# BreakTheBeta/Zonos_Vibes

Measured on AMD Instinct MI355X. Metric: real-time factor (44kHz audio s/compute s) + DAC tokens/s/GPU, Zonos-transformer, higher is better.
Workload: dtype bf16; 1 GPU; C2: batch=1 per GPU, Lc=160, 861 frames (10.00 s audio), greedy + rep. penalty, EOS suppressed, + DAC decode; global_batch=1, seq_len=1030, parallelism=dp1 (utterance-sharded), decode_steps=869

## Files before the change

include/zonos_hip.h:

```cpp
#ifndef ZONOS_HIP_H
#define ZONOS_HIP_H
#include <stdint.h>

#ifdef __cplusplus
extern "C" {
#endif

enum {
  ZMI_EPI_STORE = 0,
  ZMI_EPI_RESIDUAL = 1,
  ZMI_EPI_QKV = 2,
  ZMI_EPI_SWIGLU = 3,
  ZMI_EPI_LOGITS = 4,
  ZMI_EPI_F32 = 5
};
enum { ZMI_PACK_IDENTITY = 0, ZMI_PACK_SWIGLU = 1 };
enum { ZMI_PRO_AUTO = 0, ZMI_PRO_ADDLN = 2, ZMI_PRO_GRMS = 3, ZMI_PRO_GRMS_G = 4 };
enum { ZMI_WFMT_BF16 = 0, ZMI_WFMT_FP8 = 1 };

typedef struct ZmiGemvArgs {
  const void* W;
  const void* X;
  int M, N, K, ldx;
  int groups;
// ... 30 lines not shown
  int n_cb, n_rt, rpw;
} ZmiGemvForm;
int zmi_gemv_form(const ZmiGemvArgs* args, int epi, ZmiGemvForm* out);
int zmi_gemv_splitk(const ZmiGemvArgs* args, int epi, float* part, int64_t part_floats, void* stream);
int zmi_gemv_splitk_ln(const ZmiGemvArgs* args, int epi, float* part, int64_t part_floats, const void* ln_w,
                       const void* ln_b, float eps, void* xn, int ldxn, void* stream);
int64_t zmi_gemv_splitk_floats(int M, int N);
int zmi_layernorm_rows(const void* x, int ldx, int m, int k, const void* w, const void* b, float eps, void* out,
                       int ldo, void* stream);

int zmi_attention(const void* q, int ldq, const void* k_cache, const void* v_cache, const int* q_kv_row,
                  const int* q_pos, int n_query, int hq, int hkv, int hd, int smax, int max_pos, void* out,
                  int ldo, float* part_o, float* part_lm, void* work, void* stream);
int zmi_attention_variant(const void* q, int ldq, const void* k_cache, const void* v_cache, const int* q_kv_row,
                          const int* q_pos, int n_query, int hq, int hkv, int hd, int smax, int max_pos, void* out,
                          int ldo, float* part_o, float* part_lm, void* work, int variant, void* stream);
int zmi_attention_max_keys_whole(void);
int zmi_attention_pick(int n_query, int hkv, int variant);
int zmi_attn_block(const ZmiGemvArgs* qkv, void* gran, unsigned* err, void* attn_out, int ldo, int slices,
                   void* stream);
enum { ZMI_ATTNBLK_SELF = 256, ZMI_ATTNBLK_SPLIT = 512 };
int zmi_attn_block_max_pos(int slices);
int64_t zmi_attn_block_gran_words(int rows, int hkv);
typedef struct ZmiPrefetch {
  const void* ptr[2];
  int64_t bytes[2];
  unsigned* sink;
  int blocks, reserved;
} ZmiPrefetch;
int zmi_attn_block_pf(const ZmiGemvArgs* qkv, void* gran, unsigned* err, void* attn_out, int ldo, int slices,
                      const ZmiPrefetch* prefetch, void* stream);
int zmi_attn_block_oproj(const ZmiGemvArgs* qkv, const ZmiGemvArgs* oproj, void* gran, unsigned* err, void* attn_out,
                         int ldo, int slices, const ZmiPrefetch* prefetch, void* stream);
int zmi_attention_pf(const void* q, int ldq, const void* k_cache, const void* v_cache, const int* q_kv_row,
                     const int* q_pos, int n_query, int hq, int hkv, int hd, int smax, int max_pos, void* out, int ldo,
                     float* part_o, float* part_lm, void* work, int variant, const ZmiPrefetch* prefetch,
                     void* stream);
int64_t zmi_attention_work_bytes(int n_query, int hq, int hkv, int hd, int max_pos);
int64_t zmi_attention_partial_floats(int n_query, int hq, int hkv, int hd, int max_pos);
int zmi_attention_chunk(void);
typedef struct ZmiAttnSeq { int q_row0, len, kv_row, pos0; } ZmiAttnSeq;
typedef struct ZmiAttnTile { int seq, off; } ZmiAttnTile;
int zmi_attention_prefill(const void* q, int ldq, const void* k_cache, const void* v_cache, const ZmiAttnSeq* seqs,
                          int n_seq, int64_t n_tiles, const ZmiAttnTile* tiles, const ZmiAttnSeq* seqs_host, int hq,
                          int hkv, int hd, int smax, void* out, int ldo, void* stream);
int zmi_attention_prefill_queries(int hq, int hkv);

typedef struct ZmiSampling {
  float temperature, top_p, min_p, linear, conf, quad, rep_penalty, cfg_scale;
  int top_k, rep_window;
  uint64_t seed;
} ZmiSampling;

typedef struct ZmiSlots {
  int* active;
  int* pos;
  int* offset;
  int* remaining;
  int* stopping;
  int* step;
  int* delayed;
  const ZmiSampling* params;
  const int* total_len;
  int tcap;
  int n_slots;
} ZmiSlots;
// ... 123 lines not shown
  void* conv_ring;
  void* ssm;
  void* y;
  int ldy, gz_g;
  const int* row_pos;
  const int* row_kv;
  float* gz;
} ZmiMamba2Args;
int zmi_mamba2_step(const ZmiMamba2Args* args, void* stream);
int zmi_mamba2_scan(const ZmiMamba2Args* args, int seq_len, void* stream);
int zmi_mamba2_scan_ws(const ZmiMamba2Args* args, int seq_len, void* ws, int64_t ws_bytes, void* stream);
int64_t zmi_mamba2_scan_ws_bytes(int m, int d_ssm, int nheads);
int zmi_mamba2_scan_seqs(const ZmiMamba2Args* args, const ZmiAttnSeq* seqs, int n_seq, const ZmiAttnSeq* seqs_host,
                         void* ws, int64_t ws_bytes, void* stream);
int zmi_add_layernorm(const void* hidden, int ldh, void* residual, int ldr, int m, int k, const void* w,
                      const void* b, float eps, void* out, int ldo, int store_residual, void* stream);
int zmi_gated_rmsnorm(const void* y, int ldy, const void* z, int ldz, int m, int k, const void* w, float eps,
                      void* out, int ldo, void* stream);
int zmi_mamba_block(const ZmiGemvArgs* in_proj, const ZmiMamba2Args* step, void* gran, unsigned* err, void* stream);
int64_t zmi_mamba_block_gran_words(int rows, int d_in_proj);
int zmi_mamba_block_pf(const ZmiGemvArgs* in_proj, const ZmiMamba2Args* step, void* gran, unsigned* err,
                       const ZmiPrefetch* prefetch, void* stream);

int zmi_fill_uniform(void* dst, int64_t n, uint64_t key, float scale, float offset, int dtype, void* stream);

int zmi_graph_begin(void* stream);
int zmi_graph_end(void* stream, void** graph_exec);
int zmi_graph_launch(void* graph_exec, int times, void* stream);
int zmi_graph_destroy(void* graph_exec);

const char* zmi_last_error(void);
int zmi_version(void);
int zmi_xcd_dealing(void* stream);
enum { ZMI_OPT_GEMV_SPREAD = 0, ZMI_OPT_GEMM_ROWS = 1, ZMI_OPT_XC_HANDOFF = 2,
       ZMI_OPT_DAC_WIDE = 10, ZMI_OPT_DAC_WIDE_MIN = 11, ZMI_OPT_ATTNBLK_SPREAD = 12, ZMI_OPT_DAC_STAGE = 13,
       ZMI_OPT_DAC_STAGE_MIN = 14, ZMI_OPT_SCAN_PQ = 15, ZMI_OPT_SPLITK_WGS = 16, ZMI_OPT_SPLITK_STAGE = 17,
       ZMI_OPT_COUNT = 18 };
int zmi_set_option(int which, int value);
int zmi_get_option(int which);

#ifdef __cplusplus
}
#endif
#endif
```

zonos_vibes_amd/_lib.py:

```python
from __future__ import annotations

import ctypes
import os

HERE = os.path.dirname(os.path.abspath(__file__))
LIB_PATH = os.environ.get("ZMI_LIB_PATH") or os.path.join(HERE, "libzonos_hip.so")

c_int, c_int64, c_float, c_void_p, c_uint64 = ctypes.c_int, ctypes.c_int64, ctypes.c_float, ctypes.c_void_p, \
    ctypes.c_uint64
c_int_p = ctypes.POINTER(ctypes.c_int)

EPI_STORE, EPI_RESIDUAL, EPI_QKV, EPI_SWIGLU, EPI_LOGITS, EPI_F32 = range(6)
OPT_GEMV_SPREAD = 0
OPT_GEMM_ROWS = 1
OPT_XC_HANDOFF = 2
OPT_DAC_WIDE = 10
OPT_DAC_WIDE_MIN = 11
OPT_ATTNBLK_SPREAD = 12
OPT_DAC_STAGE = 13
OPT_DAC_STAGE_MIN = 14
OPT_SCAN_PQ = 15
OPT_SPLITK_WGS = 16
OPT_SPLITK_STAGE = 17
ATTNBLK_SELF, ATTNBLK_SPLIT = 256, 512
PACK_IDENTITY, PACK_SWIGLU = 0, 1
PRO_AUTO, PRO_ADDLN, PRO_GRMS, PRO_GRMS_G = 0, 2, 3, 4
WFMT_BF16, WFMT_FP8 = 0, 1


class GemvArgs(ctypes.Structure):
    _fields_ = [
        ("W", c_void_p), ("X", c_void_p),
        ("M", c_int), ("N", c_int), ("K", c_int), ("ldx", c_int),
        ("groups", c_int), ("reserved", c_int),
        ("ln_w", c_void_p), ("ln_b", c_void_p), ("eps", c_float),
        ("out", c_void_p), ("ldo", c_int), ("n_valid", c_int),
        ("row_kv", c_void_p), ("row_pos", c_void_p),
        ("k_cache", c_void_p), ("v_cache", c_void_p),
        ("smax", c_int), ("hq", c_int), ("hkv", c_int), ("hd", c_int),
        ("rope", c_void_p), ("diag", c_void_p),
        ("pro", c_int), ("ld_aux", c_int), ("aux", c_void_p), ("res_out", c_void_p),
        ("w_fmt", c_int), ("reserved2", c_int), ("w_exp", c_void_p),
    ]


FORM_BODY, FORM_ROWS, FORM_ROWS_DENSE = 0, 1, 2


# ... 48 lines not shown
class Mamba2Args(ctypes.Structure):
    _fields_ = [
        ("zxbcdt", c_void_p), ("ld_zx", c_int), ("M", c_int),
        ("d_ssm", c_int), ("nheads", c_int), ("headdim", c_int), ("d_state", c_int), ("d_conv", c_int),
        ("ngroups", c_int),
        ("conv_w", c_void_p), ("conv_b", c_void_p), ("dt_bias", c_void_p), ("A", c_void_p), ("D", c_void_p),
        ("conv_ring", c_void_p), ("ssm", c_void_p), ("y", c_void_p), ("ldy", c_int), ("gz_g", c_int),
        ("row_pos", c_void_p), ("row_kv", c_void_p), ("gz", c_void_p),
    ]


COND_EMBED, COND_VECTOR, COND_FOURIER, COND_LINEAR, COND_PASSTHROUGH = range(5)


_SIGS = {
    "zmi_pack_weight": (c_int, [c_void_p, c_void_p, c_int, c_int, c_int, c_int, c_void_p]),
    "zmi_gemv_launch": (c_int, [ctypes.POINTER(GemvArgs), c_int, c_void_p]),
    "zmi_gemv_form": (c_int, [ctypes.POINTER(GemvArgs), c_int, ctypes.POINTER(GemvForm)]),
    "zmi_layernorm_rows": (c_int, [c_void_p, c_int, c_int, c_int, c_void_p, c_void_p, c_float, c_void_p, c_int,
                                   c_void_p]),
    "zmi_attention": (c_int, [c_void_p, c_int, c_void_p, c_void_p, c_void_p, c_void_p, c_int, c_int, c_int, c_int,
                              c_int, c_int, c_void_p, c_int, c_void_p, c_void_p, c_void_p, c_void_p]),
    "zmi_attention_variant": (c_int, [c_void_p, c_int, c_void_p, c_void_p, c_void_p, c_void_p, c_int, c_int, c_int,
                                      c_int, c_int, c_int, c_void_p, c_int, c_void_p, c_void_p, c_void_p, c_int,
                                      c_void_p]),
    "zmi_attention_pf": (c_int, [c_void_p, c_int, c_void_p, c_void_p, c_void_p, c_void_p, c_int, c_int, c_int, c_int,
                                 c_int, c_int, c_void_p, c_int, c_void_p, c_void_p, c_void_p, c_int,
                                 ctypes.POINTER(Prefetch), c_void_p]),
    "zmi_attention_max_keys_whole": (c_int, []),
    "zmi_attention_pick": (c_int, [c_int, c_int, c_int]),
    "zmi_attn_block_max_pos": (c_int, [c_int]),
    "zmi_attn_block": (c_int, [ctypes.POINTER(GemvArgs), c_void_p, c_void_p, c_void_p, c_int, c_int, c_void_p]),
    "zmi_attn_block_gran_words": (c_int64, [c_int, c_int]),
    "zmi_gemv_splitk": (c_int, [ctypes.POINTER(GemvArgs), c_int, c_void_p, c_int64, c_void_p]),
    "zmi_gemv_splitk_floats": (c_int64, [c_int, c_int]),
    "zmi_gemv_splitk_ln": (c_int, [ctypes.POINTER(GemvArgs), c_int, c_void_p, c_int64, c_void_p, c_void_p, c_float,
                                   c_void_p, c_int, c_void_p]),
    "zmi_attn_block_pf": (c_int, [ctypes.POINTER(GemvArgs), c_void_p, c_void_p, c_void_p, c_int, c_int,
                                  ctypes.POINTER(Prefetch), c_void_p]),
    "zmi_attn_block_oproj": (c_int, [ctypes.POINTER(GemvArgs), ctypes.POINTER(GemvArgs), c_void_p, c_void_p, c_void_p,
                                     c_int, c_int, ctypes.POINTER(Prefetch), c_void_p]),
    "zmi_attention_work_bytes": (c_int64, [c_int, c_int, c_int, c_int, c_int]),
    "zmi_attention_partial_floats": (c_int64, [c_int, c_int, c_int, c_int, c_int]),
    "zmi_attention_chunk": (c_int, []),
    "zmi_attention_prefill": (c_int, [c_void_p, c_int, c_void_p, c_void_p, c_void_p, c_int, c_int64, c_void_p, c_void_p,
                                      c_int, c_int, c_int, c_int, c_void_p, c_int, c_void_p]),
    "zmi_attention_prefill_queries": (c_int, [c_int, c_int]),
    "zmi_sample_step": (c_int, [ctypes.POINTER(Slots), c_void_p, c_void_p, c_void_p, c_void_p, c_int, c_int, c_int,
                                c_void_p, c_int, c_void_p, c_void_p, c_void_p, c_void_p]),
    "zmi_sample_step_greedy": (c_int, [ctypes.POINTER(Slots), c_void_p, c_void_p, c_int, c_int, c_void_p, c_int,
                                       c_void_p, c_void_p, c_void_p, c_void_p]),
    "zmi_sample_logits": (c_int, [c_void_p, c_void_p, c_int, c_int, c_void_p, c_void_p, c_void_p, c_void_p]),
    "zmi_apply_delay_pattern": (c_int, [c_void_p, c_void_p, c_int, c_int, c_int64, c_void_p]),
    "zmi_revert_delay_pattern": (c_int, [c_void_p, c_void_p, c_int, c_int, c_void_p]),
    "zmi_embed_step": (c_int, [ctypes.POINTER(Slots), c_void_p, c_int, c_void_p, c_void_p, c_void_p, c_void_p]),
    "zmi_embed_codes": (c_int, [c_void_p, c_int, c_int, c_void_p, c_int, c_void_p, c_int, c_void_p]),
    "zmi_delay_init": (c_int, [ctypes.POINTER(Slots), c_int, c_void_p, c_int, c_int, c_void_p]),
    "zmi_delay_revert": (c_int, [ctypes.POINTER(Slots), c_int, c_void_p, c_int, c_void_p]),
    "zmi_delay_revert_range": (c_int, [ctypes.POINTER(Slots), c_int, c_int, c_int, c_void_p, c_void_p]),
    "zmi_dac_from_codes": (c_int, [c_void_p, c_int, c_void_p, c_void_p, c_void_p, c_void_p, c_void_p]),
    "zmi_dac_conv": (c_int, [c_void_p, c_int, c_int, c_void_p, c_void_p, c_int, c_int, c_int, c_int, c_int, c_int,
                             c_int, c_int, c_void_p, c_void_p, c_void_p, c_void_p, c_void_p, c_void_p]),
    "zmi_dac_from_codes_lanes": (c_int, [c_void_p, c_int, c_void_p, c_void_p, c_void_p, c_void_p, c_int, c_int64,
                                         c_int64, c_void_p]),
    "zmi_dac_conv_lanes": (c_int, [c_void_p, c_int, c_int, c_void_p, c_void_p, c_int, c_int, c_int, c_int, c_int, c_int,
                                   c_int, c_int, c_void_p, c_void_p, c_void_p, c_void_p, c_void_p, c_int, c_int64,
# ... 32 lines not shown
    "zmi_spk_simam_lanes": (c_int, [c_void_p, c_void_p, c_int, ctypes.POINTER(SpkLanes), c_int, c_void_p,
                                    ctypes.POINTER(c_int), c_void_p, c_void_p, c_int64, c_int64, c_int64, c_int64,
                                    c_int64, c_void_p]),
    "zmi_prefix_condition": (c_int, [c_void_p, c_void_p, c_int, c_void_p, c_int, c_void_p, c_void_p, c_float,
                                     c_void_p, c_void_p]),
    "zmi_mamba2_step": (c_int, [ctypes.POINTER(Mamba2Args), c_void_p]),
    "zmi_mamba2_scan": (c_int, [ctypes.POINTER(Mamba2Args), c_int, c_void_p]),
    "zmi_mamba2_scan_ws": (c_int, [ctypes.POINTER(Mamba2Args), c_int, c_void_p, ctypes.c_int64, c_void_p]),
    "zmi_mamba2_scan_ws_bytes": (ctypes.c_int64, [c_int, c_int, c_int]),
    "zmi_mamba2_scan_seqs": (c_int, [ctypes.POINTER(Mamba2Args), c_void_p, c_int, c_void_p, c_void_p, ctypes.c_int64,
                                     c_void_p]),
    "zmi_add_layernorm": (c_int, [c_void_p, c_int, c_void_p, c_int, c_int, c_int, c_void_p, c_void_p, c_float,
                                  c_void_p, c_int, c_int, c_void_p]),
    "zmi_mamba_block": (c_int, [ctypes.POINTER(GemvArgs), ctypes.POINTER(Mamba2Args), c_void_p, c_void_p, c_void_p]),
    "zmi_mamba_block_pf": (c_int, [ctypes.POINTER(GemvArgs), ctypes.POINTER(Mamba2Args), c_void_p, c_void_p,
                                   ctypes.POINTER(Prefetch), c_void_p]),
    "zmi_mamba_block_gran_words": (c_int64, [c_int, c_int]),
    "zmi_gated_rmsnorm": (c_int, [c_void_p, c_int, c_void_p, c_int, c_int, c_int, c_void_p, c_float, c_void_p, c_int,
                                  c_void_p]),
    "zmi_fill_uniform": (c_int, [c_void_p, c_int64, c_uint64, c_float, c_float, c_int, c_void_p]),
    "zmi_graph_begin": (c_int, [c_void_p]),
    "zmi_graph_end": (c_int, [c_void_p, ctypes.POINTER(c_void_p)]),
    "zmi_graph_launch": (c_int, [c_void_p, c_int, c_void_p]),
    "zmi_graph_destroy": (c_int, [c_void_p]),
    "zmi_last_error": (ctypes.c_char_p, []),
    "zmi_version": (c_int, []),
    "zmi_xcd_dealing": (c_int, [c_void_p]),
    "zmi_set_option": (c_int, [c_int, c_int]),
    "zmi_get_option": (c_int, [c_int]),
}

EXPORTED = sorted(_SIGS)
_lib = None
ABI_VERSION = 9


def load(path: str = LIB_PATH) -> ctypes.CDLL:
    import torch
    if not os.path.exists(path):
        raise RuntimeError(f"{path} is missing: build it with `python -m zonos_vibes_amd.build` "
                           "(the HIP path has no CPU fallback)")
    lib_ = ctypes.CDLL(path)
    for name, (res, args) in _SIGS.items():
        fn = getattr(lib_, name)
        fn.restype = res
        fn.argtypes = args
    if lib_.zmi_version() != ABI_VERSION:
        raise RuntimeError(f"{path} has ABI version {lib_.zmi_version()}, this binding expects {ABI_VERSION}: rebuild it")
    return lib_


def lib() -> ctypes.CDLL:
    global _lib
    if _lib is None:
        _lib = load()
    return _lib


def check(rc: int, what: str = "") -> None:
    if rc != 0:
        msg = lib().zmi_last_error().decode(errors="replace")
        raise RuntimeError(f"libzonos_hip {what} failed (status {rc}): {msg}")


def capture(stream: int, run) -> int:
    check(lib().zmi_graph_begin(stream), "graph_begin")
    try:
# ... 26 lines not shown
```

zonos_vibes_amd/csrc/zmi_attn_ds.h:

```cpp

#pragma once
#include "zmi_common.h"
#include "zmi_kernels.h"
#include "zmi_attn_merge.h"

#ifdef ZMI_ATTN_STAMPS
#define ZMI_ASTAMP(i)                                                                                    \
  do {                                                                                                   \
    if (threadIdx.x == 0 && a.stamps) a.stamps[(size_t)blockIdx.x * 8 + (i)] = __builtin_amdgcn_s_memrealtime(); \
  } while (0)
#else
#define ZMI_ASTAMP(i) \
  do {                \
  } while (0)
#endif

namespace zmi_attn {

struct AttnArgs {
  const bf16_t* q;
  int ldq;
  const bf16_t* k;
  const bf16_t* v;
  const int* kv_row;
  const int* pos;
  int hkv, smax, nch;
  float scale;
  bf16_t* out;
  int ldo;
  unsigned* err;
  unsigned* tickets;
  uint64_t* gran;
  float* part_o;
  float* part_lm;
  unsigned long long* stamps;
  ZmiPrefetch pf;
  int n_att, n_pf;
  int xc_l2;
};

__device__ __forceinline__ f32x4_t mfma16(const uint4& a, const uint4& b, f32x4_t c) {
  return __builtin_amdgcn_mfma_f32_16x16x32_bf16(__builtin_bit_cast(bf16x8_t, a), __builtin_bit_cast(bf16x8_t, b), c,
                                                 0, 0, 0);
}

constexpr int DNW = 8;
constexpr int DKM = 5;
constexpr int DS_KEYS = 32 * DNW * DKM;
constexpr int DS_CH = DS_KEYS / CH;
constexpr int DS_BLK = (DS_KEYS + BLK - 1) / BLK;
constexpr unsigned DS_SPIN_LIMIT = 1u << 18;

template <int G, int DS>
struct DsImg {
  static constexpr int DSD = HD / DS;
  static constexpr int NG = DNW * DKM;
  static constexpr size_t SC = 0;
  static constexpr size_t PB = SC + (size_t)G * DS_KEYS * 4;
  static constexpr size_t OP = PB + (size_t)G * DS_KEYS * 2;
  static constexpr size_t MJ = OP + (size_t)NG * G * DSD * 4;
  static constexpr size_t LJ = MJ + (size_t)DS_CH * G * 4;
  static constexpr size_t MB = LJ + (size_t)DS_CH * G * 4;
  static constexpr size_t BYTES = (MB + (size_t)DS_BLK * G * 4 + 15) / 16 * 16;
};

template <int G, int DS, int W0 = 0, int NWK = DNW, int VR = DKM>
__device__ __forceinline__ void ds_tail(const AttnArgs& a, char* smem, uint4 (&vf)[VR][8 / DS], int qi, int kh,
                                        int s, int pos) {
  constexpr int CPG = CH / 32;
  constexpr int DT = 8 / DS;
  using I = DsImg<G, DS>;
// ... 202 lines not shown
```

zonos_vibes_amd/csrc/zmi_attnblk.hip:

```cpp
#include <algorithm>

#include "zmi_common.h"
#include "zmi_kernels.h"
#include "zmi_gemv_impl.h"
#include "zmi_prefetch.h"
#include "zmi_attn_ds.h"

namespace {

using namespace zmi_attn;
constexpr int QG = 2, QW = 4, QNL = 8, QRT = 16;
static_assert(QG * QW == DNW, "both roles run the same block size");
constexpr int XG = 4;
constexpr int QKV_GRAN = (XG + 2) * HD / 2;
constexpr int XC_CH_MAX = 24;
constexpr int XC_WORDS_MAX = 3 * XC_CH_MAX * XG + XC_CH_MAX * XG * HD + XG * HD / 2 + HD / 16;
constexpr int GRAN_STRIDE = QKV_GRAN + (XG * DS_KEYS > XC_WORDS_MAX ? XG * DS_KEYS : XC_WORDS_MAX);
constexpr int NT = DNW * 64;
constexpr unsigned XS_SPIN = 1u << 16;

__device__ __forceinline__ uint32_t tag_of(uint64_t g) { return (uint32_t)(g >> 32); }

__device__ __forceinline__ void give_up(const AttnArgs& a) {
  __hip_atomic_store(a.err, 1u, __ATOMIC_RELAXED, __HIP_MEMORY_SCOPE_AGENT);
}

constexpr int XNWK = DNW - 1;
constexpr int XCH = DS_KEYS / CH;
constexpr int XRC = (XCH + XNWK - 1) / XNWK;
constexpr int CPG = CH / 32;
constexpr int XKPT = (DS_KEYS + NT - 1) / NT;

template <int S>
struct XsImg {
  static constexpr int DSD = HD / S;
  static constexpr size_t SC = 0;
  static constexpr size_t PB = SC + (size_t)XG * DS_KEYS * 4;
  static constexpr size_t OC = PB + (size_t)XG * DS_KEYS * 2;
  static constexpr size_t MJ = OC + (size_t)XCH * XG * DSD * 4;
  static constexpr size_t LJ = MJ + (size_t)XCH * XG * 4;
  static constexpr size_t MB = LJ + (size_t)XCH * XG * 4;
  static constexpr size_t QKV = MB + (size_t)DS_BLK * XG * 4;
  static constexpr size_t BYTES = (QKV + (size_t)QKV_GRAN * 4 + 15) / 16 * 16;
};

template <int S>
__device__ __forceinline__ void xs_body(const AttnArgs& a, int n_units, int b, char* smem, uint64_t* gran) {
  constexpr int OWN = (DS_KEYS / 32 + S - 1) / S;
  constexpr int KPW = (OWN + XNWK - 1) / XNWK;
// ... 620 lines not shown
      if (cc >= nc) break;
      const float o = ocv[cc];
      if (cc % CPB == 0) {
        ob = o;
        lb = lcv[cc];
        mb = mblk[cc / CPB][g];
      } else {
        ob += o;
        lb += lcv[cc];
      }
      if (cc % CPB == CPB - 1 || cc == nc - 1) {
        if (cc < CPB) {
          acc = ob;
          l = lb;
        } else {
          const float et = expf(mprev - mb);
          l = lb + et * l;
          acc = acc * et + ob;
        }
        mprev = mb;
      }
    }
    const float rl = 1.0f / l;
    a.out[(size_t)qi * a.ldo + (kh * XG + g) * HD + DSD * s + dl] = (bf16_t)f2bf(acc * rl);
  }
  ZMI_ASTAMP(6);
}

template <int XCH>
struct XcG {
  static constexpr int KEYS = XCH * CH;
  static constexpr int GM = 0, GL = GM + XCH * XG, GB = GL + XCH * XG, GO = GB + XCH * XG;
  static constexpr int WORDS = GO + XCH * XG * HD;
  static constexpr int OG = WORDS, OF = OG + XG * HD / 2, OWORDS = OF + HD / 16;
  static constexpr bool OPROJ_FITS = QKV_GRAN + OWORDS <= GRAN_STRIDE;
  static_assert(WORDS <= GRAN_STRIDE - QKV_GRAN, "the chunk-split granules fit the unit's area");
  static_assert(XCH >= HD / 16 && XCH % CPB == 0 && XCH <= XC_CH_MAX, "8 merging workgroups; whole 512-key blocks");
};
constexpr int XC_KEYS = XcG<8>::KEYS;
static_assert(CH == 128 && DNW == 8, "eight waves: one 16-key score tile each over a 128-key chunk");

struct XcImg {
  static constexpr size_t SC = 0;
  static constexpr size_t PB = SC + (size_t)XG * CH * 4;
  static constexpr size_t OP = PB + (size_t)XG * CH * 2;
  static constexpr size_t MJ = OP + (size_t)CPG * XG * HD * 4;
  static constexpr size_t QKV = MJ + (size_t)XG * 4;
  static constexpr size_t BYTES = (QKV + (size_t)QKV_GRAN * 4 + 15) / 16 * 16;
};

#ifndef ZMI_XC_QKV_SLEEP
#define ZMI_XC_QKV_SLEEP 2
#endif
template <int XCH, bool OPROJ>
__device__ __forceinline__ void xc_body(const AttnArgs& a, int n_units, int b, char* smem, uint64_t* gran) {
  using X = XcG<XCH>;
  constexpr int XC_CH = XCH, XC_GM = X::GM, XC_GL = X::GL, XC_GB = X::GB, XC_GO = X::GO;
  float(&sc)[XG][CH] = *reinterpret_cast<float(*)[XG][CH]>(smem + XcImg::SC);
  bf16_t(&pb)[XG][CH] = *reinterpret_cast<bf16_t(*)[XG][CH]>(smem + XcImg::PB);
  float(&opart)[CPG][XG][HD] = *reinterpret_cast<float(*)[CPG][XG][HD]>(smem + XcImg::OP);
  float* mj = reinterpret_cast<float*>(smem + XcImg::MJ);
  uint32_t* qkv_lds = reinterpret_cast<uint32_t*>(smem + XcImg::QKV);

  const int y = b >> 3;
  const int c = y % XC_CH, unit = 8 * (y / XC_CH) + (b & 7);
  if (unit >= n_units) return;
  const int qi = unit / a.hkv, kh = unit - qi * a.hkv;
// ... 221 lines not shown
    if (wave < NBLK && wave * CPB < nc) pend |= 1u << (2 * KPW);
    for (unsigned spins = 0; pend; ++spins) {
#pragma unroll
      for (int i = 0; i < KPW; ++i) {
        const int k = wave + DNW * i;
        if ((pend >> (2 * i)) & 1) ov[i] = ld_wt64(gx + XC_GO + (k * XG + g) * HD + d);
        if ((pend >> (2 * i + 1)) & 1) lv[i] = ld_wt64(gx + XC_GL + k * XG + g);
      }
      if ((pend >> (2 * KPW)) & 1) mv = ld_wt64(gx + XC_GB + wave * CPB * XG + g);
#pragma unroll
      for (int i = 0; i < KPW; ++i) {
        if (((pend >> (2 * i)) & 1) && tag_of(ov[i]) == tag) pend &= ~(1u << (2 * i));
        if (((pend >> (2 * i + 1)) & 1) && tag_of(lv[i]) == tag) pend &= ~(1u << (2 * i + 1));
      }
      if (((pend >> (2 * KPW)) & 1) && tag_of(mv) == tag) pend &= ~(1u << (2 * KPW));
      if (__all(pend == 0)) break;
      if (spins > XS_SPIN) {
        give_up(a);
        break;
      }
      __builtin_amdgcn_s_sleep(2);
    }
#pragma unroll
    for (int i = 0; i < KPW; ++i) {
      const int k = wave + DNW * i;
      if (k < nc) {
        mO[k * (XG * 16) + l64] = __uint_as_float((uint32_t)ov[i]);
        if ((l64 & 15) == 0) mL[k * XG + g] = __uint_as_float((uint32_t)lv[i]);
      }
    }
    if (wave < NBLK && wave * CPB < nc && (l64 & 15) == 0) mM[wave * XG + g] = __uint_as_float((uint32_t)mv);
    __syncthreads();
  }
  if (c < HD / 16 && t < XG * 16) {
    const int g = t >> 4, d = 16 * c + (t & 15);
    const float* mO = reinterpret_cast<const float*>(smem + XcImg::OP);
    const float* mL = reinterpret_cast<const float*>(smem + XcImg::SC);
    const float* mM = mL + XC_CH * XG;
    float acc = 0.f, l = 0.f, ob = 0.f, lb = 0.f, mprev = 0.f, mb = 0.f;
    for (int k = 0; k < nc; ++k) {
      const float o = mO[k * (XG * 16) + t], lk = mL[k * XG + g];
      if (k % CPB == 0) {
        ob = o;
        lb = lk;
        mb = mM[(k / CPB) * XG + g];
      } else {
        ob += o;
        lb += lk;
      }
      if (k % CPB == CPB - 1 || k == nc - 1) {
        if (k < CPB) {
          acc = ob;
          l = lb;
        } else {
          const float et = expf(mprev - mb);
          l = lb + et * l;
          acc = acc * et + ob;
        }
        mprev = mb;
      }
    }
    const float rl = 1.0f / l;
    const uint32_t ov16 = f2bf(acc * rl);
    a.out[(size_t)qi * a.ldo + (kh * XG + g) * HD + d] = (bf16_t)ov16;
    if constexpr (OPROJ) {
      static_assert(X::OPROJ_FITS, "the output granules fit the unit's area");
      const uint32_t nb = (uint32_t)__shfl_xor((int)ov16, 1);
      if ((t & 1) == 0) st_wt64(gu + QKV_GRAN + X::OG + ((g * HD + d) >> 1), (uint64_t)(ov16 | (nb << 16)) | tag64);
      if (t == 0) st_wt64(gu + QKV_GRAN + X::OF + c, tag64);
    }
  }
  ZMI_ASTAMP(6);
}

template <int S, int PRO, int FORM, bool OPROJ>
__global__ __launch_bounds__(NT) void attn_block_kernel(const ZmiGemvArgs qa, int n_cb, int n_qkv, const AttnArgs at,
                                                        int n_units, uint64_t* gran, const ZmiPrefetch pf, int n_pf,
                                                        const ZmiGemvArgs oa, int n_op) {
  extern __shared__ __attribute__((aligned(16))) char smem[];
  const int b = blockIdx.x;
  const int n_xs = (n_units + 7) / 8 * 8 * S;
  if (b < n_qkv)
    zmi_gemv::gemv_body<QG, QW, QNL, QRT, PRO, ZMI_EPI_QKV, 1, 1>(
        qa, n_cb, 1, b, smem, zmi_gemv::QkvFuse{gran, GRAN_STRIDE});
  else if (b < n_qkv + n_xs) {
    if constexpr (FORM == FORM_SELF)
      xr_body<S>(at, n_units, b - n_qkv, smem, gran);
    else if constexpr (FORM == FORM_SPLIT)
      xc_body<S, OPROJ>(at, n_units, b - n_qkv, smem, gran);
    else
      xs_body<S>(at, n_units, b - n_qkv, smem, gran);
  } else if (OPROJ && b < n_qkv + n_xs + n_op) {
    if constexpr (OPROJ) {
      using X = XcG<S>;
      zmi_gemv::QkvFuse fz{gran, GRAN_STRIDE};
      fz.og_off = QKV_GRAN + X::OG;
      fz.of_off = QKV_GRAN + X::OF;
      fz.hkv = at.hkv;
      fz.pos = at.pos;
      fz.err = at.err;
      constexpr int OEPI = PRO == zmi_gemv::PRO_ADDLN ? ZMI_EPI_STORE : ZMI_EPI_RESIDUAL;
      zmi_gemv::gemv_body<QG, QW, QNL, QRT, zmi_gemv::PRO_PLAIN, OEPI, 1, 3>(oa, oa.N / 8 / QG, 1, b - n_qkv - n_xs,
                                                                             smem, fz);
    }
  } else
    prefetch_body<NT>(pf, b - n_qkv - n_xs - n_op, n_pf);
}

template <int S, int PRO, int FORM, bool OPROJ = false>
hipError_t launch_block(const ZmiGemvArgs& a, int n_cb, int n_qkv, const AttnArgs& at, int n_units, uint64_t* gran,
                        const ZmiPrefetch& pf, hipStream_t s, const ZmiGemvArgs* oa = nullptr) {
  const int fl = (zmi_option(ZMI_OPT_ATTNBLK_SPREAD) >> (S == 24 ? 2 : 0)) & 3;
  const size_t spread = fl == 1 ? zmi_gemv::LDS_MAX / 2 + 1024 : (fl == 2 ? zmi_gemv::LDS_MAX / 3 + 1024 : 0);
  const size_t lds = std::max({zmi_gemv::Img<2048>::bytes(a.M, DNW, QRT, PRO),
                               FORM == FORM_SELF ? XrImg<S>::BYTES : (FORM == FORM_SPLIT ? XcImg::BYTES : XsImg<S>::BYTES),
                               spread});
  if (lds > zmi_gemv::LDS_MAX) return hipErrorInvalidValue;
  if (lds > 64 * 1024) {
    static const hipError_t attr = hipFuncSetAttribute(
        reinterpret_cast<const void*>(&attn_block_kernel<S, PRO, FORM, OPROJ>), hipFuncAttributeMaxDynamicSharedMemorySize,
        (int)zmi_gemv::LDS_MAX);
    if (attr != hipSuccess) return attr;
  }
  const int n_xs = (n_units + 7) / 8 * 8 * S;
  const int n_pf = (pf.bytes[0] > 0 || pf.bytes[1] > 0) ? pf.blocks : 0;
  const int n_op = OPROJ ? (oa->N / 8 / QG + 7) / 8 * 8 : 0;
  hipLaunchKernelGGL((attn_block_kernel<S, PRO, FORM, OPROJ>), dim3((unsigned)(n_qkv + n_xs + n_op + n_pf)), dim3(NT),
                     lds, s, a, n_cb, n_qkv, at, n_units, gran, pf, n_pf, OPROJ ? *oa : a, n_op);
  return hipGetLastError();
}

}

extern "C" int64_t zmi_attn_block_gran_words(int rows, int hkv) {
  return (rows <= 0 || hkv <= 0) ? -1 : (int64_t)rows * hkv * GRAN_STRIDE;
}

namespace {
int attn_block(const ZmiGemvArgs* qkv, const ZmiGemvArgs* oproj, void* gran, unsigned* err, void* attn_out, int ldo,
               int slices, const ZmiPrefetch* prefetch, void* stream) {
  const ZmiGemvArgs& a = *qkv;
  if (a.K != 2048 || !a.ln_w) return zmi_fail_msg("attn_block: the QKV projection must be LayerNorm'd with K = 2048");
  if (a.w_fmt != ZMI_WFMT_BF16 || (oproj && oproj->w_fmt != ZMI_WFMT_BF16))
    return zmi_fail_msg("attn_block: bf16 weights only");
  const bool addln = a.pro == ZMI_PRO_ADDLN;
  if (a.pro != ZMI_PRO_AUTO && !addln) return zmi_fail_msg("attn_block: prologue must be LayerNorm or ADDLN");
  if (addln && (!a.ln_b || !a.aux || a.ld_aux % 8 || a.res_out == a.aux))
    return zmi_fail_msg("attn_block: ADDLN needs ln_b, the residual rows (ld_aux % 8) and a separate res_out");
  if (a.M < 1 || a.M > QRT) return zmi_fail_msg("attn_block: 1 <= M <= 16 rows (one row tile)");
  if (a.hd != HD || a.hkv <= 0 || a.hq != XG * a.hkv)
    return zmi_fail_msg("attn_block: head_dim 128, 4 query heads per kv head");
  if (a.N != (a.hq + 2 * a.hkv) * a.hd || a.n_valid != a.N) return zmi_fail_msg("attn_block: N = (hq + 2 hkv) hd");
  if (a.smax % 8 || !a.row_pos || !a.row_kv || !a.rope || !a.k_cache || !a.v_cache || !gran || !err || !attn_out)
    return zmi_fail_msg("attn_block: missing buffers (or smax % 8)");
  if (ldo % 8 || a.ldx % 8) return zmi_fail_msg("attn_block: ldo / ldx must be multiples of 8");
  const int n_cb = a.N / 8 / QG;
  const int n_qkv = (n_cb + 7) / 8 * 8;
  const int n_units = a.M * a.hkv;

  AttnArgs at{};
  at.q = (const bf16_t*)a.out;
  at.ldq = a.ldo;
  at.k = (const bf16_t*)a.k_cache;
  at.v = (const bf16_t*)a.v_cache;
  at.kv_row = a.row_kv;
  at.pos = a.row_pos;
  at.hkv = a.hkv;
  at.smax = a.smax;
  at.scale = 1.0f / sqrtf((float)HD);
  at.out = (bf16_t*)attn_out;
  at.ldo = ldo;
  at.err = err;
  at.xc_l2 = zmi_option(ZMI_OPT_XC_HANDOFF) == 0 ? 1 : 0;
  at.stamps = a.diag ? reinterpret_cast<unsigned long long*>(a.diag) + (size_t)a.reserved * 4096 * 8 : nullptr;
  ZmiPrefetch pf{};
  if (prefetch) {
    pf = *prefetch;
    if (zmi_prefetch_invalid(pf)) return zmi_fail_msg("attn_block: bad prefetch ranges");
  }
  hipStream_t s = (hipStream_t)stream;
  hipError_t e;
  using zmi_gemv::PRO_ADDLN;
  using zmi_gemv::PRO_LN;
  const int form = (slices & ZMI_ATTNBLK_SPLIT) ? FORM_SPLIT : ((slices & ZMI_ATTNBLK_SELF) ? FORM_SELF : FORM_XS);
  const int sl = slices & ~(ZMI_ATTNBLK_SELF | ZMI_ATTNBLK_SPLIT);
  if (form == FORM_SPLIT ? (sl != 8 && sl != 24) : (sl != 4 && sl != 8))
    return zmi_fail_msg("attn_block: slices must be 4 or 8 (| ZMI_ATTNBLK_SELF), or 8 or 24 | ZMI_ATTNBLK_SPLIT");
  if (oproj) {
    const ZmiGemvArgs& o = *oproj;
    if (form != FORM_SPLIT)
      return zmi_fail_msg("attn_block: the fused out_proj runs with the chunk-split forms");
    if (o.K != a.hq * a.hd || o.N % (8 * QG) || o.n_valid != o.N || o.M != a.M || o.ln_w || o.pro != ZMI_PRO_AUTO ||
        !o.out || o.ldo % 8 || o.ldo < o.N || o.X != attn_out)
      return zmi_fail_msg("attn_block: out_proj must be the plain residual GEMV over the attention output "
                          "(K = hq hd, N % 16 == 0, same rows, X = attn_out)");
    if (addln && (o.out == a.aux || o.out == a.res_out))
      return zmi_fail_msg("attn_block: the ADDLN block's out_proj writes the hidden rows, not the residual buffers");
    if (sl == 8)
      ZMI_CHECK(addln ? (launch_block<8, zmi_gemv::PRO_ADDLN, FORM_SPLIT, true>(a, n_cb, n_qkv, at, n_units,
                                                                                 (uint64_t*)gran, pf, s, oproj))
                      : (launch_block<8, zmi_gemv::PRO_LN, FORM_SPLIT, true>(a, n_cb, n_qkv, at, n_units, (uint64_t*)gran,
                                                                              pf, s, oproj)));
    else
      ZMI_CHECK(addln ? (launch_block<24, zmi_gemv::PRO_ADDLN, FORM_SPLIT, true>(a, n_cb, n_qkv, at, n_units,
                                                                                  (uint64_t*)gran, pf, s, oproj))
                      : (launch_block<24, zmi_gemv::PRO_LN, FORM_SPLIT, true>(a, n_cb, n_qkv, at, n_units, (uint64_t*)gran,
// ... 38 lines not shown
```

zonos_vibes_amd/csrc/zmi_gemv_impl.h:

```cpp
#pragma once
#include <algorithm>
#include "zmi_common.h"
#include "zmi_kernels.h"
#include "zmi_gemv_row.h"

namespace zmi_gemv {

constexpr int PRO_PLAIN = 0, PRO_LN = 1, PRO_ADDLN = 2, PRO_GRMS = 3;
constexpr int PRO_GRMSG = 4;
constexpr size_t LDS_MAX = 160 * 1024;

__device__ __forceinline__ void dma_piece(const bf16_t* gsrc, bf16_t* ldp) {
  const unsigned ldst =
      __builtin_amdgcn_readfirstlane((unsigned)(size_t)(__attribute__((address_space(3))) void*)ldp);
  unsigned keep;
  asm volatile("s_mov_b32 %0, m0\n\ts_mov_b32 m0, %2\n\ts_nop 0\n\tglobal_load_lds_dwordx4 %1, off\n\t"
               "s_mov_b32 m0, %0"
               : "=&s"(keep)
               : "v"(gsrc), "s"(ldst)
               : "memory");
}

template <int K>
struct Img {
// ... 34 lines not shown
      t += d0 * d0 + d1 * d1;
    } else {
      t += s0 + s1;
    }
  }
  return t;
}
__device__ __forceinline__ float gate_elem(const uint32_t (&y)[4], const float (&gz)[8], int e) {
  return bf2f(y[e >> 1] >> (16 * (e & 1))) * gz[e];
}
__device__ __forceinline__ void load_gate(const float* p, float (&gz)[8]) {
  const float4 a = *reinterpret_cast<const float4*>(p), b = *reinterpret_cast<const float4*>(p + 4);
  gz[0] = a.x; gz[1] = a.y; gz[2] = a.z; gz[3] = a.w; gz[4] = b.x; gz[5] = b.y; gz[6] = b.z; gz[7] = b.w;
}

#ifdef ZMI_GEMV_STAMPS
#define ZMI_GSTAMP(i)                                                                              \
  do {                                                                                             \
    __builtin_amdgcn_sched_barrier(0);                                                             \
    if (threadIdx.x == 0 && a.diag)                                                                \
      reinterpret_cast<unsigned long long*>(a.diag)[((size_t)a.reserved * 4096 + blockIdx.x) * 8 + (i)] = \
          __builtin_amdgcn_s_memrealtime();                                                        \
    __builtin_amdgcn_sched_barrier(0);                                                             \
  } while (0)
#else
#define ZMI_GSTAMP(i) \
  do {                \
  } while (0)
#endif

struct QkvFuse {
  uint64_t* gran;
  int gran_stride;
  int og_off = 0, of_off = 0, hkv = 0;
  const int* pos = nullptr;
  unsigned* err = nullptr;
  int l2_cols = 0;
};

__device__ __forceinline__ const float2* rope_pair(const ZmiGemvArgs& a, int q_pos, int n) {
  const int qcols = a.hq * a.hd, d = (n < qcols ? n : n - qcols) % a.hd;
  return reinterpret_cast<const float2*>(a.rope + ((size_t)q_pos * (a.hd >> 1) + (d >> 1)) * 2);
}

template <int EPI, int RT, int FUSE, class Sum>
__device__ __forceinline__ void epilogue(const ZmiGemvArgs& a, const Sum& colsum, int lane, int rows, int row0,
                                         int g, const uint32_t (&res_pre)[(8 * RT + 63) / 64], int q_pos, int q_kvr,
                                         const QkvFuse& fz, unsigned act_rows = ~0u, const float2* rope_pre = nullptr) {
  constexpr int NE = (8 * RT + 63) / 64;
  const int col0 = g * 8;
  if (EPI == ZMI_EPI_STORE && FUSE == 2) {
#pragma unroll
    for (int i = 0; i < NE; ++i) {
      const int e = lane + 64 * i, r = e >> 3, c = e & 7, n = col0 + c;
      const bool ok = r < rows && n < a.n_valid;
      const uint32_t hv = ok ? f2bf(colsum(c, r)) : 0u;
      const uint32_t nb = (uint32_t)__shfl_down((int)hv, 1);
      if (ok) {
        const size_t m = (size_t)(row0 + r);
        reinterpret_cast<bf16_t*>(a.out)[m * a.ldo + n] = (bf16_t)hv;
        const int pos = a.row_pos[m];
        if ((c & 1) == 0 && pos >= 0)
          st_xc64(fz.gran + m * fz.gran_stride + (n >> 1), (uint64_t)(hv | (nb << 16)) | ((uint64_t)(unsigned)(pos + 1) << 32),
                  n < fz.l2_cols);
      }
    }
  } else if (EPI == ZMI_EPI_STORE || EPI == ZMI_EPI_RESIDUAL || EPI == ZMI_EPI_F32 || EPI == ZMI_EPI_LOGITS) {
// ... 99 lines not shown

template <int EPI, int RT>
__device__ __forceinline__ void stage_epilogue_operands(const ZmiGemvArgs& a, bool ew, int lane, int rows, int row0,
                                                        int col0, uint32_t (&res_pre)[(8 * RT + 63) / 64], int& q_pos,
                                                        int& q_kvr) {
  constexpr int NE = (8 * RT + 63) / 64;
#pragma unroll
  for (int i = 0; i < NE; ++i) res_pre[i] = 0;
  q_pos = -1, q_kvr = 0;
  if (EPI == ZMI_EPI_RESIDUAL && ew) {
#pragma unroll
    for (int i = 0; i < NE; ++i) {
      const int e = lane + 64 * i, r = e >> 3, n = col0 + (e & 7);
      if (r < rows && n < a.n_valid)
        res_pre[i] = reinterpret_cast<const bf16_t*>(a.out)[(size_t)(row0 + r) * a.ldo + n];
    }
  }
  if (EPI == ZMI_EPI_QKV && ew && (lane >> 2) < rows) {
    q_pos = a.row_pos[row0 + (lane >> 2)];
    q_kvr = a.row_kv[row0 + (lane >> 2)];
  }
}

template <int K, int NWV>
__device__ __forceinline__ unsigned gather_attention_rows(const ZmiGemvArgs& a, const QkvFuse& fz, bf16_t* xs, int* qpos,
                                                          int rows, int row0, int tid) {
  constexpr int XROW = Img<K>::XROW;
  const int lane = tid & 63, wave = __builtin_amdgcn_readfirstlane(tid >> 6);
  if (tid < rows) qpos[tid] = fz.pos[row0 + tid];
  __syncthreads();
  unsigned act_rows = 0u;
  for (int r = 0; r < rows; ++r) act_rows |= (qpos[r] >= 0 ? 1u : 0u) << r;
  const int n_units = rows * fz.hkv;
  if (wave == 0) {
    for (unsigned spins = 0;; ++spins) {
      bool ok = false;
      for (int u0 = 0; u0 < n_units; u0 += 8) {
        const int u = u0 + (lane >> 3), qp = u < n_units ? qpos[u / fz.hkv] : -1;
        const bool up = qp < 0 || (uint32_t)(ld_wt64(fz.gran + (size_t)(row0 * fz.hkv + u) * fz.gran_stride + fz.of_off +
                                                        (lane & 7)) >> 32) == (uint32_t)qp + 1u;
        float f = up ? 1.f : 0.f;
        f = fmaxf(f, dpp_mov<DPP_XOR1>(f));
        f = fmaxf(f, dpp_mov<DPP_XOR2>(f));
        f = fmaxf(f, dpp_mov<DPP_HALF_MIRROR>(f));
        ok = ok || (u < n_units && f > 0.f);
      }
      if (__any(ok)) break;
      if (spins > (1u << 18)) {
        if (lane == 0) __hip_atomic_store(fz.err, 1u, __ATOMIC_RELAXED, __HIP_MEMORY_SCOPE_AGENT);
        break;
      }
      __builtin_amdgcn_s_sleep(2);
    }
  }
  ZMI_GSTAMP(7);
  __syncthreads();
  constexpr int GPT = 4;
  for (int e0 = tid; e0 < n_units * 256; e0 += GPT * NWV * 64) {
    uint64_t gv[GPT];
    int gq[GPT];
    unsigned need = 0;
#pragma unroll
    for (int i = 0; i < GPT; ++i) {
      const int e = e0 + NWV * 64 * i;
      gq[i] = e < n_units * 256 ? qpos[(e >> 8) / fz.hkv] : -1;
      gv[i] = 0ull;
      if (gq[i] >= 0) need |= 1u << i;
    }
    for (unsigned spins = 0; need; ++spins) {
#pragma unroll
      for (int i = 0; i < GPT; ++i)
        if ((need >> i) & 1)
          gv[i] = ld_wt64(fz.gran + (size_t)(row0 * fz.hkv + ((e0 + NWV * 64 * i) >> 8)) * fz.gran_stride + fz.og_off +
                          ((e0 + NWV * 64 * i) & 255));
#pragma unroll
      for (int i = 0; i < GPT; ++i)
        if (((need >> i) & 1) && (uint32_t)(gv[i] >> 32) == (uint32_t)gq[i] + 1u) need &= ~(1u << i);
      if (!need) break;
      if (spins > (1u << 18)) {
        __hip_atomic_store(fz.err, 1u, __ATOMIC_RELAXED, __HIP_MEMORY_SCOPE_AGENT);
        break;
      }
      __builtin_amdgcn_s_sleep(1);
    }
#pragma unroll
    for (int i = 0; i < GPT; ++i) {
      const int e = e0 + NWV * 64 * i;
      if (e < n_units * 256) {
        const int u = e >> 8, j = e & 255, r = u / fz.hkv, kh = u - r * fz.hkv;
        *reinterpret_cast<uint32_t*>(xs + r * XROW + kh * 512 + 2 * j) = gq[i] >= 0 ? (uint32_t)gv[i] : 0u;
      }
    }
  }
  return act_rows;
}

template <int K, int RT, int NWV, bool ADD>
__device__ __forceinline__ void ln_statistics(const ZmiGemvArgs& a, const View<K>& L, int rows, int wave, int lane) {
  constexpr int XROW = Img<K>::XROW, NQ = ln_parts(K), CPQ = K / (512 * NQ);
  float* part = L.red;
  const int ntask = rows * NQ;
  auto pass = [&](int task, float mean, bool sq) {
    const int r = task / NQ, q = task - r * NQ;
    const int off = r * XROW + q * (K / NQ) + lane * 8;
    float t = 0.f;
#pragma unroll
// ... 619 lines not shown
```

zonos_vibes_amd/csrc/zmi_misc.hip:

```cpp
#include <stdio.h>
#include <string.h>

#include "zmi_common.h"
#include "zmi_kernels.h"

static thread_local char g_err[512] = "";

int zmi_fail(hipError_t e, const char* what, const char* file, int line) {
  snprintf(g_err, sizeof(g_err), "%s failed: %s (%s:%d)", what, hipGetErrorString(e), file, line);
  return (int)e == 0 ? -1 : (int)e;
}

int zmi_fail_msg(const char* msg) {
  snprintf(g_err, sizeof(g_err), "%s", msg);
  return -1;
}

extern "C" const char* zmi_last_error(void) { return g_err; }
extern "C" int zmi_version(void) { return 9; }

static int g_opts[ZMI_OPT_COUNT] = {1, 3, 0, 0, 1, 8, 2, 1, 1, 0, 1, 256, 5, 29, 128, 0, 256, 1};
int zmi_option(int which) { return (which >= 0 && which < ZMI_OPT_COUNT) ? g_opts[which] : 0; }
extern "C" int zmi_set_option(int which, int value) {
  if (which < 0 || which >= ZMI_OPT_COUNT) return zmi_fail_msg("zmi_set_option: unknown option");
  g_opts[which] = value;
  return 0;
}
extern "C" int zmi_get_option(int which) { return zmi_option(which); }
static int g_cus = 0;
int zmi_cu_count() {
  if (!g_cus) {
    int dev = 0, n = 0;
    if (hipGetDevice(&dev) == hipSuccess && hipDeviceGetAttribute(&n, hipDeviceAttributeMultiprocessorCount, dev) == hipSuccess && n > 0)
      g_cus = n;
    else
      g_cus = 256;
  }
  return g_cus;
}

namespace {
__global__ void xcc_kernel(unsigned* xcc) {
  unsigned v;
  asm volatile("s_getreg_b32 %0, hwreg(HW_REG_XCC_ID)" : "=s"(v));
  if (threadIdx.x == 0) xcc[blockIdx.x] = v;
}
}

extern "C" int zmi_xcd_dealing(void* stream) {
  constexpr int NB = 1024;
  unsigned* d = nullptr;
  unsigned h[NB];
// ... 134 lines not shown
```

Before: 12.78 x realtime (audio s / wall s, all GPUs).

## Replicate attention output granules per XCD for the fused o-proj gather

The attention merge stage now writes its output granules and ready flags into eight separate copies, one per wave, instead of a single shared area. Each o-proj GEMV workgroup polls and reads the copy picked by blockIdx & 7, which tracks the XCD it runs on. The aim is to spread the flag spinning and granule reads across distinct cache lines, so the cross-XCD handoff between attention and o-proj is less contended. In exchange, the merge is recomputed redundantly by up to eight waves, there are more write-through stores, and the granule area grows; an option restores the single-copy path.

```diff
diff --git a/include/zonos_hip.h b/include/zonos_hip.h
--- a/include/zonos_hip.h
+++ b/include/zonos_hip.h
@@ -86,6 +86,7 @@
                       const ZmiPrefetch* prefetch, void* stream);
 int zmi_attn_block_oproj(const ZmiGemvArgs* qkv, const ZmiGemvArgs* oproj, void* gran, unsigned* err, void* attn_out,
                          int ldo, int slices, const ZmiPrefetch* prefetch, void* stream);
+int zmi_attn_block_oproj_layout(int slices, int* og_word, int* copy_stride, int* copies);
 int zmi_attention_pf(const void* q, int ldq, const void* k_cache, const void* v_cache, const int* q_kv_row,
                      const int* q_pos, int n_query, int hq, int hkv, int hd, int smax, int max_pos, void* out, int ldo,
                      float* part_o, float* part_lm, void* work, int variant, const ZmiPrefetch* prefetch,
@@ -275,7 +276,7 @@
 const char* zmi_last_error(void);
 int zmi_version(void);
 int zmi_xcd_dealing(void* stream);
-enum { ZMI_OPT_GEMV_SPREAD = 0, ZMI_OPT_GEMM_ROWS = 1, ZMI_OPT_XC_HANDOFF = 2,
+enum { ZMI_OPT_GEMV_SPREAD = 0, ZMI_OPT_GEMM_ROWS = 1, ZMI_OPT_XC_HANDOFF = 2, ZMI_OPT_OPROJ_GATHER = 3,
        ZMI_OPT_DAC_WIDE = 10, ZMI_OPT_DAC_WIDE_MIN = 11, ZMI_OPT_ATTNBLK_SPREAD = 12, ZMI_OPT_DAC_STAGE = 13,
        ZMI_OPT_DAC_STAGE_MIN = 14, ZMI_OPT_SCAN_PQ = 15, ZMI_OPT_SPLITK_WGS = 16, ZMI_OPT_SPLITK_STAGE = 17,
        ZMI_OPT_COUNT = 18 };
diff --git a/zonos_vibes_amd/_lib.py b/zonos_vibes_amd/_lib.py
--- a/zonos_vibes_amd/_lib.py
+++ b/zonos_vibes_amd/_lib.py
@@ -14,6 +14,7 @@
 OPT_GEMV_SPREAD = 0
 OPT_GEMM_ROWS = 1
 OPT_XC_HANDOFF = 2
+OPT_OPROJ_GATHER = 3
 OPT_DAC_WIDE = 10
 OPT_DAC_WIDE_MIN = 11
 OPT_ATTNBLK_SPREAD = 12
@@ -128,6 +129,7 @@
     "zmi_attn_block_max_pos": (c_int, [c_int]),
     "zmi_attn_block": (c_int, [ctypes.POINTER(GemvArgs), c_void_p, c_void_p, c_void_p, c_int, c_int, c_void_p]),
     "zmi_attn_block_gran_words": (c_int64, [c_int, c_int]),
+    "zmi_attn_block_oproj_layout": (c_int, [c_int, c_int_p, c_int_p, c_int_p]),
     "zmi_gemv_splitk": (c_int, [ctypes.POINTER(GemvArgs), c_int, c_void_p, c_int64, c_void_p]),
     "zmi_gemv_splitk_floats": (c_int64, [c_int, c_int]),
     "zmi_gemv_splitk_ln": (c_int, [ctypes.POINTER(GemvArgs), c_int, c_void_p, c_int64, c_void_p, c_void_p, c_float,
@@ -226,7 +228,7 @@
 
 EXPORTED = sorted(_SIGS)
 _lib = None
-ABI_VERSION = 9
+ABI_VERSION = 10
 
 
 def load(path: str = LIB_PATH) -> ctypes.CDLL:
diff --git a/zonos_vibes_amd/csrc/zmi_attn_ds.h b/zonos_vibes_amd/csrc/zmi_attn_ds.h
--- a/zonos_vibes_amd/csrc/zmi_attn_ds.h
+++ b/zonos_vibes_amd/csrc/zmi_attn_ds.h
@@ -37,6 +37,7 @@
   ZmiPrefetch pf;
   int n_att, n_pf;
   int xc_l2;
+  int og_copies;
 };
 
 __device__ __forceinline__ f32x4_t mfma16(const uint4& a, const uint4& b, f32x4_t c) {
diff --git a/zonos_vibes_amd/csrc/zmi_attnblk.hip b/zonos_vibes_amd/csrc/zmi_attnblk.hip
--- a/zonos_vibes_amd/csrc/zmi_attnblk.hip
+++ b/zonos_vibes_amd/csrc/zmi_attnblk.hip
@@ -14,7 +14,10 @@
 constexpr int XG = 4;
 constexpr int QKV_GRAN = (XG + 2) * HD / 2;
 constexpr int XC_CH_MAX = 24;
-constexpr int XC_WORDS_MAX = 3 * XC_CH_MAX * XG + XC_CH_MAX * XG * HD + XG * HD / 2 + HD / 16;
+constexpr int OG_COPIES = 8;
+constexpr int OG_COPY_WORDS = 512;
+static_assert(OG_COPY_WORDS >= XG * HD / 2 + HD / 16, "a copy holds the output granules and the flags");
+constexpr int XC_WORDS_MAX = 3 * XC_CH_MAX * XG + XC_CH_MAX * XG * HD + OG_COPIES * OG_COPY_WORDS;
 constexpr int GRAN_STRIDE = QKV_GRAN + (XG * DS_KEYS > XC_WORDS_MAX ? XG * DS_KEYS : XC_WORDS_MAX);
 constexpr int NT = DNW * 64;
 constexpr unsigned XS_SPIN = 1u << 16;
@@ -701,7 +704,7 @@
   static constexpr int KEYS = XCH * CH;
   static constexpr int GM = 0, GL = GM + XCH * XG, GB = GL + XCH * XG, GO = GB + XCH * XG;
   static constexpr int WORDS = GO + XCH * XG * HD;
-  static constexpr int OG = WORDS, OF = OG + XG * HD / 2, OWORDS = OF + HD / 16;
+  static constexpr int OG = WORDS, OF = OG + XG * HD / 2, OWORDS = OG + OG_COPIES * OG_COPY_WORDS;
   static constexpr bool OPROJ_FITS = QKV_GRAN + OWORDS <= GRAN_STRIDE;
   static_assert(WORDS <= GRAN_STRIDE - QKV_GRAN, "the chunk-split granules fit the unit's area");
   static_assert(XCH >= HD / 16 && XCH % CPB == 0 && XCH <= XC_CH_MAX, "8 merging workgroups; whole 512-key blocks");
@@ -989,14 +992,14 @@
     if (wave < NBLK && wave * CPB < nc && (l64 & 15) == 0) mM[wave * XG + g] = __uint_as_float((uint32_t)mv);
     __syncthreads();
   }
-  if (c < HD / 16 && t < XG * 16) {
-    const int g = t >> 4, d = 16 * c + (t & 15);
+  if (c < HD / 16 && wave < (OPROJ ? a.og_copies : 1)) {
+    const int l64 = t & 63, g = l64 >> 4, d = 16 * c + (l64 & 15);
     const float* mO = reinterpret_cast<const float*>(smem + XcImg::OP);
     const float* mL = reinterpret_cast<const float*>(smem + XcImg::SC);
     const float* mM = mL + XC_CH * XG;
     float acc = 0.f, l = 0.f, ob = 0.f, lb = 0.f, mprev = 0.f, mb = 0.f;
     for (int k = 0; k < nc; ++k) {
-      const float o = mO[k * (XG * 16) + t], lk = mL[k * XG + g];
+      const float o = mO[k * (XG * 16) + l64], lk = mL[k * XG + g];
       if (k % CPB == 0) {
         ob = o;
         lb = lk;
@@ -1019,12 +1022,13 @@
     }
     const float rl = 1.0f / l;
     const uint32_t ov16 = f2bf(acc * rl);
-    a.out[(size_t)qi * a.ldo + (kh * XG + g) * HD + d] = (bf16_t)ov16;
+    if (wave == 0) a.out[(size_t)qi * a.ldo + (kh * XG + g) * HD + d] = (bf16_t)ov16;
     if constexpr (OPROJ) {
-      static_assert(X::OPROJ_FITS, "the output granules fit the unit's area");
+      static_assert(X::OPROJ_FITS && OG_COPIES <= DNW, "the output granules fit the unit's area; one copy per wave");
       const uint32_t nb = (uint32_t)__shfl_xor((int)ov16, 1);
-      if ((t & 1) == 0) st_wt64(gu + QKV_GRAN + X::OG + ((g * HD + d) >> 1), (uint64_t)(ov16 | (nb << 16)) | tag64);
-      if (t == 0) st_wt64(gu + QKV_GRAN + X::OF + c, tag64);
+      uint64_t* oc = gu + QKV_GRAN + X::OG + wave * OG_COPY_WORDS;
+      if ((l64 & 1) == 0) st_wt64(oc + ((g * HD + d) >> 1), (uint64_t)(ov16 | (nb << 16)) | tag64);
+      if (l64 == 0) st_wt64(oc + (X::OF - X::OG) + c, tag64);
     }
   }
   ZMI_ASTAMP(6);
@@ -1053,6 +1057,8 @@
       zmi_gemv::QkvFuse fz{gran, GRAN_STRIDE};
       fz.og_off = QKV_GRAN + X::OG;
       fz.of_off = QKV_GRAN + X::OF;
+      fz.og_copies = at.og_copies;
+      fz.og_copy_stride = OG_COPY_WORDS;
       fz.hkv = at.hkv;
       fz.pos = at.pos;
       fz.err = at.err;
@@ -1091,6 +1097,15 @@
 
 extern "C" int64_t zmi_attn_block_gran_words(int rows, int hkv) {
   return (rows <= 0 || hkv <= 0) ? -1 : (int64_t)rows * hkv * GRAN_STRIDE;
+}
+
+extern "C" int zmi_attn_block_oproj_layout(int slices, int* og_word, int* copy_stride, int* copies) {
+  const int sl = slices & ~ZMI_ATTNBLK_SPLIT;
+  if (sl != 8 && sl != 24) return zmi_fail_msg("attn_block_oproj_layout: slices must be 8 or 24 (| ZMI_ATTNBLK_SPLIT)");
+  if (og_word) *og_word = QKV_GRAN + (sl == 8 ? XcG<8>::OG : XcG<24>::OG);
+  if (copy_stride) *copy_stride = OG_COPY_WORDS;
+  if (copies) *copies = OG_COPIES;
+  return 0;
 }
 
 namespace {
@@ -1129,6 +1144,7 @@
   at.ldo = ldo;
   at.err = err;
   at.xc_l2 = zmi_option(ZMI_OPT_XC_HANDOFF) == 0 ? 1 : 0;
+  at.og_copies = zmi_option(ZMI_OPT_OPROJ_GATHER) == 0 ? OG_COPIES : 1;
   at.stamps = a.diag ? reinterpret_cast<unsigned long long*>(a.diag) + (size_t)a.reserved * 4096 * 8 : nullptr;
   ZmiPrefetch pf{};
   if (prefetch) {
diff --git a/zonos_vibes_amd/csrc/zmi_gemv_impl.h b/zonos_vibes_amd/csrc/zmi_gemv_impl.h
--- a/zonos_vibes_amd/csrc/zmi_gemv_impl.h
+++ b/zonos_vibes_amd/csrc/zmi_gemv_impl.h
@@ -90,7 +90,7 @@
 struct QkvFuse {
   uint64_t* gran;
   int gran_stride;
-  int og_off = 0, of_off = 0, hkv = 0;
+  int og_off = 0, of_off = 0, hkv = 0, og_copies = 1, og_copy_stride = 0;
   const int* pos = nullptr;
   unsigned* err = nullptr;
   int l2_cols = 0;
@@ -256,12 +256,13 @@
   unsigned act_rows = 0u;
   for (int r = 0; r < rows; ++r) act_rows |= (qpos[r] >= 0 ? 1u : 0u) << r;
   const int n_units = rows * fz.hkv;
+  const uint64_t* gc = fz.gran + (size_t)((int)(blockIdx.x & 7u) % fz.og_copies) * fz.og_copy_stride;
   if (wave == 0) {
     for (unsigned spins = 0;; ++spins) {
       bool ok = false;
       for (int u0 = 0; u0 < n_units; u0 += 8) {
         const int u = u0 + (lane >> 3), qp = u < n_units ? qpos[u / fz.hkv] : -1;
-        const bool up = qp < 0 || (uint32_t)(ld_wt64(fz.gran + (size_t)(row0 * fz.hkv + u) * fz.gran_stride + fz.of_off +
+        const bool up = qp < 0 || (uint32_t)(ld_wt64(gc + (size_t)(row0 * fz.hkv + u) * fz.gran_stride + fz.of_off +
                                                         (lane & 7)) >> 32) == (uint32_t)qp + 1u;
         float f = up ? 1.f : 0.f;
         f = fmaxf(f, dpp_mov<DPP_XOR1>(f));
@@ -295,7 +296,7 @@
 #pragma unroll
       for (int i = 0; i < GPT; ++i)
         if ((need >> i) & 1)
-          gv[i] = ld_wt64(fz.gran + (size_t)(row0 * fz.hkv + ((e0 + NWV * 64 * i) >> 8)) * fz.gran_stride + fz.og_off +
+          gv[i] = ld_wt64(gc + (size_t)(row0 * fz.hkv + ((e0 + NWV * 64 * i) >> 8)) * fz.gran_stride + fz.og_off +
                           ((e0 + NWV * 64 * i) & 255));
 #pragma unroll
       for (int i = 0; i < GPT; ++i)
diff --git a/zonos_vibes_amd/csrc/zmi_misc.hip b/zonos_vibes_amd/csrc/zmi_misc.hip
--- a/zonos_vibes_amd/csrc/zmi_misc.hip
+++ b/zonos_vibes_amd/csrc/zmi_misc.hip
@@ -17,7 +17,7 @@
 }
 
 extern "C" const char* zmi_last_error(void) { return g_err; }
-extern "C" int zmi_version(void) { return 9; }
+extern "C" int zmi_version(void) { return 10; }
 
 static int g_opts[ZMI_OPT_COUNT] = {1, 3, 0, 0, 1, 8, 2, 1, 1, 0, 1, 256, 5, 29, 128, 0, 256, 1};
 int zmi_option(int which) { return (which >= 0 && which < ZMI_OPT_COUNT) ? g_opts[which] : 0; }
```

Measured after the change: 12.77 x realtime (audio s / wall s, all GPUs), median of 3. About the same (-0.1%).
